# awsaf49/vip-cup-2022

Hardware: AMD Instinct MI355X
Metric: images/sec (200x200, full ensemble) (higher is better)
Workload: dtype f16; 1 GPU; ensemble8; precision=fast, distinct_images=5120, global_batch=256, parallelism=image-parallel dp1, one all-gather of scores, member_streams=3

## Files before the change

### vip-cup-2022_amd/csrc/mlp_fused.hip

```cpp
#include "common.hpp"

namespace {

struct MlpArgs {
    const f16* x;
    const f16* w1;
    const float* b1;
    const f16* w2;
    const float* b2;
    const f16* res;
    f16* y;
    const float* ln_g;
    const float* ln_b;
    float ln_eps;
    int M, Hd;
    int ldx, ldy, ldr, ldw1, ldw2;
    long x_bytes, y_bytes, res_bytes;
    int s1, s2;
    int n_tiles;
};

__device__ __forceinline__ int frag_channel(int j) {
    const int t = (j >> 4) & 1, r = j & 15;
    return (j & ~31) + (r >> 2) * 8 + t * 4 + (r & 3);
}


template <int CK>
__device__ __forceinline__ void ln_fragments(U4H8 (&xf)[CK], const float* __restrict__ g, const float* __restrict__ b,
                                             float eps, int lq) {
    constexpr int C = 32 * CK;
    float v[CK][8];
    float sum = 0.f;
#pragma unroll
    for (int ks = 0; ks < CK; ++ks)
#pragma unroll
        for (int j = 0; j < 8; ++j) {
            v[ks][j] = (float)xf[ks].e[j];
            sum += v[ks][j];
        }
    sum += __shfl_xor(sum, 16, 64);
    sum += __shfl_xor(sum, 32, 64);
    const float mean = sum / (float)C;
    float sq = 0.f;
#pragma unroll
    for (int ks = 0; ks < CK; ++ks)
#pragma unroll
        for (int j = 0; j < 8; ++j) {
            const float d = v[ks][j] - mean;
            sq += d * d;
        }
    sq += __shfl_xor(sq, 16, 64);
    sq += __shfl_xor(sq, 32, 64);
    const float rstd = rsqrtf(sq / (float)C + eps);
#pragma unroll
    for (int ks = 0; ks < CK; ++ks) {
        const float4 g0 = *reinterpret_cast<const float4*>(g + ks * 32 + lq * 8), g1 = *reinterpret_cast<const float4*>(g + ks * 32 + lq * 8 + 4);
        const float4 b0 = *reinterpret_cast<const float4*>(b + ks * 32 + lq * 8), b1 = *reinterpret_cast<const float4*>(b + ks * 32 + lq * 8 + 4);
        const float gg[8] = {g0.x, g0.y, g0.z, g0.w, g1.x, g1.y, g1.z, g1.w};
        const float bb[8] = {b0.x, b0.y, b0.z, b0.w, b1.x, b1.y, b1.z, b1.w};
#pragma unroll
        for (int j = 0; j < 8; ++j) xf[ks].e[j] = (f16)((v[ks][j] - mean) * rstd * gg[j] + bb[j]);
    }
}

template <int CK, int ACT, int PT>
__global__ __launch_bounds__(2048 / PT, 1) void mlp_fused_kernel(MlpArgs a) {
    constexpr int C = 32 * CK, NCT = C / 16, NTHR = 2048 / PT;
    constexpr unsigned OOB = 0xFFFFFFF0u;
    extern __shared__ __attribute__((aligned(16))) char smem[];
    char* w1s = smem;
    char* w2s = smem + a.Hd * a.s1;

    const int tid = threadIdx.x, lane = tid & 63, wave = tid >> 6;
    const int l15 = lane & 15, lq = lane >> 4;

    {
        const __amdgpu_buffer_rsrc_t r1 = __builtin_amdgcn_make_buffer_rsrc((void*)a.w1, 0, (unsigned)(2L * a.Hd * a.ldw1), 0x00020000);
        const __amdgpu_buffer_rsrc_t r2 = __builtin_amdgcn_make_buffer_rsrc((void*)a.w2, 0, (unsigned)(2L * C * a.ldw2), 0x00020000);
        constexpr int cpr1 = CK * 4;
        for (int i = tid; i < a.Hd * cpr1; i += NTHR) {
            const int j = i / cpr1, c = i - j * cpr1;
            const uint4 v = __builtin_bit_cast(
                uint4, __builtin_amdgcn_raw_buffer_load_b128(r1, (unsigned)((frag_channel(j) * a.ldw1 + c * 8) * 2), 0, 0));
            *reinterpret_cast<uint4*>(w1s + j * a.s1 + c * 16) = v;
        }
        const int cpr2 = a.Hd >> 3;
        for (int i = tid; i < C * cpr2; i += NTHR) {
            const int j = i / cpr2, c = i - j * cpr2;
            const uint4 v = __builtin_bit_cast(
                uint4, __builtin_amdgcn_raw_buffer_load_b128(r2, (unsigned)((frag_channel(j) * a.ldw2 + c * 8) * 2), 0, 0));
            *reinterpret_cast<uint4*>(w2s + j * a.s2 + c * 16) = v;
        }
    }
    __syncthreads();

    const __amdgpu_buffer_rsrc_t rx = __builtin_amdgcn_make_buffer_rsrc((void*)a.x, 0, (unsigned)a.x_bytes, 0x00020000);
    const __amdgpu_buffer_rsrc_t rr = __builtin_amdgcn_make_buffer_rsrc((void*)a.res, 0, a.res ? (unsigned)a.res_bytes : 0u, 0x00020000);
    const __amdgpu_buffer_rsrc_t ry = __builtin_amdgcn_make_buffer_rsrc((void*)a.y, 0, (unsigned)a.y_bytes, 0x00020000);
    const __amdgpu_buffer_rsrc_t rb1 = __builtin_amdgcn_make_buffer_rsrc((void*)a.b1, 0, a.b1 ? (unsigned)(a.Hd * 4) : 0u, 0x00020000);
    const __amdgpu_buffer_rsrc_t rb2 = __builtin_amdgcn_make_buffer_rsrc((void*)a.b2, 0, a.b2 ? (unsigned)(C * 4) : 0u, 0x00020000);
    const char* w1l = w1s + l15 * a.s1 + lq * 16;
    const char* w2l = w2s + l15 * a.s2 + lq * 16;
    const int nq = a.Hd >> 5;

    for (int tile = blockIdx.x; tile < a.n_tiles; tile += gridDim.x) {
        const int m0 = tile * 512 + wave * (16 * PT);
        U4H8 xf[CK][PT];
#pragma unroll
        for (int ks = 0; ks < CK; ++ks)
#pragma unroll
            for (int p = 0; p < PT; ++p) {
                const int m = m0 + p * 16 + l15;
                xf[ks][p].u = __builtin_bit_cast(
                    uint4, __builtin_amdgcn_raw_buffer_load_b128(rx, m < a.M ? (unsigned)((m * a.ldx + ks * 32 + lq * 8) * 2) : OOB, 0, 0));
            }
        if (a.ln_g) {
#pragma unroll
            for (int p = 0; p < PT; ++p) {
                U4H8 col[CK];
#pragma unroll
                for (int ks = 0; ks < CK; ++ks) col[ks] = xf[ks][p];
                ln_fragments<CK>(col, a.ln_g, a.ln_b, a.ln_eps, lq);
#pragma unroll
                for (int ks = 0; ks < CK; ++ks) xf[ks][p] = col[ks];
            }
        }
        f32x4 acc2[NCT][PT];
#pragma unroll
        for (int ct = 0; ct < NCT; ++ct) {
            const f32x4 bv = __builtin_bit_cast(
                f32x4, __builtin_amdgcn_raw_buffer_load_b128(rb2, (unsigned)(((ct >> 1) * 32 + lq * 8 + (ct & 1) * 4) * 4), 0, 0));
#pragma unroll
            for (int p = 0; p < PT; ++p) acc2[ct][p] = bv;
        }

        auto gemm1 = [&](int q, f32x4 (&acc1)[2][PT]) {
#pragma unroll
            for (int t = 0; t < 2; ++t) {
                const f32x4 bv = __builtin_bit_cast(
                    f32x4, __builtin_amdgcn_raw_buffer_load_b128(rb1, (unsigned)((q * 32 + lq * 8 + t * 4) * 4), 0, 0));
#pragma unroll
                for (int p = 0; p < PT; ++p) acc1[t][p] = bv;
            }
#pragma unroll
            for (int ks = 0; ks < CK; ++ks)
#pragma unroll
                for (int t = 0; t < 2; ++t) {
                    U4H8 wf;
                    wf.u = *reinterpret_cast<const uint4*>(w1l + (q * 32 + t * 16) * a.s1 + ks * 64);
#pragma unroll
                    for (int p = 0; p < PT; ++p)
                        acc1[t][p] = __builtin_amdgcn_mfma_f32_16x16x32_f16(wf.h, xf[ks][p].h, acc1[t][p], 0, 0, 0);
                }
        };
        auto act_pack = [&](const f32x4 (&acc1)[2][PT], U4H8 (&hf)[PT]) {
#pragma unroll
            for (int p = 0; p < PT; ++p)
#pragma unroll
                for (int t = 0; t < 2; ++t)
#pragma unroll
                    for (int j = 0; j < 4; j += 2) {
                        const f32x2 v = vip_act2<ACT>((f32x2){acc1[t][p][j], acc1[t][p][j + 1]});
                        hf[p].e[t * 4 + j] = (f16)v.x;
                        hf[p].e[t * 4 + j + 1] = (f16)v.y;
                    }
        };
        auto gemm2 = [&](int q, const U4H8 (&hf)[PT]) {
#pragma unroll
            for (int ct = 0; ct < NCT; ++ct) {
                U4H8 wf;
                wf.u = *reinterpret_cast<const uint4*>(w2l + ct * 16 * a.s2 + q * 64);
#pragma unroll
                for (int p = 0; p < PT; ++p)
                    acc2[ct][p] = __builtin_amdgcn_mfma_f32_16x16x32_f16(wf.h, hf[p].h, acc2[ct][p], 0, 0, 0);
            }
        };
        U4H8 hf[PT];
#pragma unroll 1
        for (int q = 0; q < nq; ++q) {
            f32x4 h0[2][PT];
            gemm1(q, h0);
            act_pack(h0, hf);
            gemm2(q, hf);
        }

#pragma unroll
        for (int p = 0; p < PT; ++p) {
            const int m = m0 + p * 16 + l15;
            const bool ok = m < a.M;
#pragma unroll
            for (int hh = 0; hh < CK; ++hh) {
                const int n = hh * 32 + lq * 8;
                U4H8 r;
                r.u = __builtin_bit_cast(uint4, __builtin_amdgcn_raw_buffer_load_b128(
                                                    rr, ok ? (unsigned)((m * a.ldr + n) * 2) : OOB, 0, 0));
                U4H8 o;
#pragma unroll
                for (int j = 0; j < 8; j += 2) {
                    const f32x4 av = acc2[2 * hh + (j >> 2)][p];
                    const f32x2 v = (f32x2){av[j & 3], av[(j & 3) + 1]} + (f32x2){(float)r.e[j], (float)r.e[j + 1]};
                    o.e[j] = (f16)v.x;
                    o.e[j + 1] = (f16)v.y;
                }
                __builtin_amdgcn_raw_buffer_store_b128(
                    __builtin_bit_cast(__attribute__((__vector_size__(4 * sizeof(unsigned)))) unsigned, o.u), ry,
                    ok ? (unsigned)((m * a.ldy + n) * 2) : OOB, 0, 0);
            }
        }
    }
}

static int mlp_stride(int chunks) {
    while ((chunks & 3) != 2) ++chunks;
    return chunks * 16;
}

static int mlp_cu_count() {
    static int n_cu = 0;
    if (!n_cu) {
        int dev = 0;
        hipDeviceProp_t prop;
        if (hipGetDevice(&dev) == hipSuccess && hipGetDeviceProperties(&prop, dev) == hipSuccess) n_cu = prop.multiProcessorCount;
        if (n_cu <= 0) n_cu = 256;
    }
    return n_cu;
}

struct MlpPlan {
    int s1, s2;
    size_t smem;
    int tile;
    int n_tiles;
    int grid;
};

static bool mlp_plan_resident(int C, int M, int Hd, MlpPlan& p) {
    p.s1 = mlp_stride(C / 8);
    p.s2 = mlp_stride(Hd >> 3);
    p.smem = (size_t)Hd * p.s1 + (size_t)C * p.s2;
    if (p.smem > 160 * 1024) return false;
    p.tile = 512;
    p.n_tiles = (M + 511) / 512;
    const int n_cu = mlp_cu_count();
    p.grid = p.n_tiles < n_cu ? p.n_tiles : n_cu;
    return true;
}

static void mlp_plan_stream(int C, int M, MlpPlan& p) {
    p.s1 = mlp_stride(C / 8);
    p.s2 = mlp_stride(4);
    p.smem = 2 * ((size_t)32 * p.s1 + (size_t)C * p.s2);
    p.tile = 256;
    p.n_tiles = (M + 255) / 256;
    const int n_cu = mlp_cu_count();
    p.grid = p.n_tiles < n_cu ? p.n_tiles : n_cu;
}

template <int CK>
int launch_mlp(MlpArgs a, hipStream_t s) {
    MlpPlan p;
    if (!mlp_plan_resident(32 * CK, a.M, a.Hd, p)) return 1;
    a.s1 = p.s1;
    a.s2 = p.s2;
    a.n_tiles = p.n_tiles;
    static bool attr_set = false;
    if (!attr_set) {
        (void)hipFuncSetAttribute(reinterpret_cast<const void*>(mlp_fused_kernel<CK, VIP_ACT_GELU, 2>),
                                  hipFuncAttributeMaxDynamicSharedMemorySize, 160 * 1024);
        attr_set = true;
    }
    hipLaunchKernelGGL((mlp_fused_kernel<CK, VIP_ACT_GELU, 2>), dim3(p.grid), dim3(1024), p.smem, s, a);
    return vip_launch_status("vip_mlp_fused_f16");
}


template <int CK, int ACT>
__global__ __launch_bounds__(512, 1) void mlp_stream_kernel(MlpArgs a) {
    constexpr int C = 32 * CK, PT = 2, NCT = C / 16, NTHR = 512;
    constexpr int W_IT = C / 64;
    constexpr unsigned OOB = 0xFFFFFFF0u;
    extern __shared__ __attribute__((aligned(16))) char smem[];
    const int stage_bytes = 32 * a.s1 + C * a.s2;

    const int tid = threadIdx.x, lane = tid & 63, wave = tid >> 6;
    const int l15 = lane & 15, lq = lane >> 4;

    const __amdgpu_buffer_rsrc_t rx = __builtin_amdgcn_make_buffer_rsrc((void*)a.x, 0, (unsigned)a.x_bytes, 0x00020000);
    const __amdgpu_buffer_rsrc_t rr = __builtin_amdgcn_make_buffer_rsrc((void*)a.res, 0, a.res ? (unsigned)a.res_bytes : 0u, 0x00020000);
    const __amdgpu_buffer_rsrc_t ry = __builtin_amdgcn_make_buffer_rsrc((void*)a.y, 0, (unsigned)a.y_bytes, 0x00020000);
    const __amdgpu_buffer_rsrc_t rb1 = __builtin_amdgcn_make_buffer_rsrc((void*)a.b1, 0, a.b1 ? (unsigned)(a.Hd * 4) : 0u, 0x00020000);
    const __amdgpu_buffer_rsrc_t rb2 = __builtin_amdgcn_make_buffer_rsrc((void*)a.b2, 0, a.b2 ? (unsigned)(C * 4) : 0u, 0x00020000);

    const char* w_ptr[W_IT];
    unsigned w_step[W_IT];
    int w_dst[W_IT];
#pragma unroll
    for (int i = 0; i < W_IT; ++i) {
        const int idx = tid + NTHR * i;
        if (idx < 4 * C) {
            const int row = idx / (C / 8), c = idx - row * (C / 8);
            w_ptr[i] = reinterpret_cast<const char*>(a.w1) + ((long)frag_channel(row) * a.ldw1 + c * 8) * 2;
            w_step[i] = (unsigned)(32 * a.ldw1 * 2);
            w_dst[i] = row * a.s1 + c * 16;
        } else {
            const int j = idx - 4 * C, row = j >> 2, c = j & 3;
            w_ptr[i] = reinterpret_cast<const char*>(a.w2) + ((long)frag_channel(row) * a.ldw2 + c * 8) * 2;
            w_step[i] = 64u;
            w_dst[i] = 32 * a.s1 + row * a.s2 + c * 16;
        }
    }
    uint4 wst[W_IT];
    auto load_w = [&](int q) {
#pragma unroll
        for (int i = 0; i < W_IT; ++i) wst[i] = *reinterpret_cast<const uint4*>(w_ptr[i] + (size_t)q * w_step[i]);
    };
    auto store_w = [&](int buf) {
#pragma unroll
        for (int i = 0; i < W_IT; ++i) *reinterpret_cast<uint4*>(smem + buf * stage_bytes + w_dst[i]) = wst[i];
    };

    const int nq = a.Hd >> 5;
    load_w(0);
    store_w(0);
    __syncthreads();
    int buf = 0;

    for (int tile = blockIdx.x; tile < a.n_tiles; tile += gridDim.x) {
        const int m0 = tile * (NTHR / 64 * 16 * PT) + wave * (16 * PT);
        U4H8 xf[CK][PT];
#pragma unroll
        for (int ks = 0; ks < CK; ++ks)
#pragma unroll
            for (int p = 0; p < PT; ++p) {
                const int m = m0 + p * 16 + l15;
                xf[ks][p].u = __builtin_bit_cast(
                    uint4, __builtin_amdgcn_raw_buffer_load_b128(rx, m < a.M ? (unsigned)((m * a.ldx + ks * 32 + lq * 8) * 2) : OOB, 0, 0));
            }
        if (a.ln_g) {
#pragma unroll
            for (int p = 0; p < PT; ++p) {
                U4H8 col[CK];
#pragma unroll
                for (int ks = 0; ks < CK; ++ks) col[ks] = xf[ks][p];
                ln_fragments<CK>(col, a.ln_g, a.ln_b, a.ln_eps, lq);
#pragma unroll
                for (int ks = 0; ks < CK; ++ks) xf[ks][p] = col[ks];
            }
        }
        f32x4 acc2[NCT][PT];
#pragma unroll
        for (int ct = 0; ct < NCT; ++ct) {
            const f32x4 bv = __builtin_bit_cast(
                f32x4, __builtin_amdgcn_raw_buffer_load_b128(rb2, (unsigned)(((ct >> 1) * 32 + lq * 8 + (ct & 1) * 4) * 4), 0, 0));
#pragma unroll
            for (int p = 0; p < PT; ++p) acc2[ct][p] = bv;
        }

#pragma unroll 1
        for (int q = 0; q < nq; ++q) {
            load_w(q + 1 < nq ? q + 1 : 0);
            __builtin_amdgcn_sched_barrier(0);
            const char* w1l = smem + buf * stage_bytes + l15 * a.s1 + lq * 16;
            const char* w2l = smem + buf * stage_bytes + 32 * a.s1 + l15 * a.s2 + lq * 16;
            f32x4 acc1[2][PT];
#pragma unroll
            for (int t = 0; t < 2; ++t) {
                const f32x4 bv = __builtin_bit_cast(
                    f32x4, __builtin_amdgcn_raw_buffer_load_b128(rb1, (unsigned)((q * 32 + lq * 8 + t * 4) * 4), 0, 0));
#pragma unroll
                for (int p = 0; p < PT; ++p) acc1[t][p] = bv;
            }
#pragma unroll
            for (int ks = 0; ks < CK; ++ks)
#pragma unroll
                for (int t = 0; t < 2; ++t) {
                    U4H8 wf;
                    wf.u = *reinterpret_cast<const uint4*>(w1l + t * 16 * a.s1 + ks * 64);
#pragma unroll
                    for (int p = 0; p < PT; ++p)
                        acc1[t][p] = __builtin_amdgcn_mfma_f32_16x16x32_f16(wf.h, xf[ks][p].h, acc1[t][p], 0, 0, 0);
                }
            U4H8 hf[PT];
#pragma unroll
            for (int p = 0; p < PT; ++p)
#pragma unroll
                for (int t = 0; t < 2; ++t)
#pragma unroll
                    for (int j = 0; j < 4; j += 2) {
                        const f32x2 v = vip_act2<ACT>((f32x2){acc1[t][p][j], acc1[t][p][j + 1]});
                        hf[p].e[t * 4 + j] = (f16)v.x;
                        hf[p].e[t * 4 + j + 1] = (f16)v.y;
                    }
#pragma unroll
            for (int ct = 0; ct < NCT; ++ct) {
                U4H8 wf;
                wf.u = *reinterpret_cast<const uint4*>(w2l + ct * 16 * a.s2);
#pragma unroll
                for (int p = 0; p < PT; ++p)
                    acc2[ct][p] = __builtin_amdgcn_mfma_f32_16x16x32_f16(wf.h, hf[p].h, acc2[ct][p], 0, 0, 0);
            }
            __builtin_amdgcn_sched_barrier(0);
            store_w(buf ^ 1);
            __syncthreads();
            buf ^= 1;
        }

#pragma unroll
        for (int p = 0; p < PT; ++p) {
            const int m = m0 + p * 16 + l15;
            const bool ok = m < a.M;
#pragma unroll
            for (int hh = 0; hh < CK; ++hh) {
                const int n = hh * 32 + lq * 8;
                U4H8 r;
                r.u = __builtin_bit_cast(uint4, __builtin_amdgcn_raw_buffer_load_b128(
                                                    rr, ok ? (unsigned)((m * a.ldr + n) * 2) : OOB, 0, 0));
                U4H8 o;
#pragma unroll
                for (int j = 0; j < 8; j += 2) {
                    const f32x4 av = acc2[2 * hh + (j >> 2)][p];
                    const f32x2 v = (f32x2){av[j & 3], av[(j & 3) + 1]} + (f32x2){(float)r.e[j], (float)r.e[j + 1]};
                    o.e[j] = (f16)v.x;
                    o.e[j + 1] = (f16)v.y;
                }
                __builtin_amdgcn_raw_buffer_store_b128(
                    __builtin_bit_cast(__attribute__((__vector_size__(4 * sizeof(unsigned)))) unsigned, o.u), ry,
                    ok ? (unsigned)((m * a.ldy + n) * 2) : OOB, 0, 0);
            }
        }
    }
}

template <int CK>
int launch_mlp_stream(MlpArgs a, hipStream_t s) {
    MlpPlan p;
    mlp_plan_stream(32 * CK, a.M, p);
    a.s1 = p.s1;
    a.s2 = p.s2;
    a.n_tiles = p.n_tiles;
    static bool attr_set = false;
    if (!attr_set) {
        (void)hipFuncSetAttribute(reinterpret_cast<const void*>(mlp_stream_kernel<CK, VIP_ACT_GELU>),
                                  hipFuncAttributeMaxDynamicSharedMemorySize, 160 * 1024);
        attr_set = true;
    }
    hipLaunchKernelGGL((mlp_stream_kernel<CK, VIP_ACT_GELU>), dim3(p.grid), dim3(512), p.smem, s, a);
    return vip_launch_status("vip_mlp_fused_f16(stream)");
}

}

extern "C" int vip_mlp_fused_supported(int M, int C, int hidden, int act) {
    if (act != VIP_ACT_GELU || hidden % 32 != 0 || hidden <= 0 || M < 8192) return 0;
    if (C == 192) return 1;
    if (C != 64 && C != 96) return 0;
    const long s1 = mlp_stride(C / 8), s2 = mlp_stride(hidden >> 3);
    return (long)hidden * s1 + (long)C * s2 <= 160 * 1024;
}

extern "C" int vip_mlp_fused_plan(int M, int C, int hidden, int act, int* workgroups, int* tile_rows) {
    if (!vip_mlp_fused_supported(M, C, hidden, act)) return 0;
    MlpPlan p;
    if (C == 192) mlp_plan_stream(C, M, p);
    else if (!mlp_plan_resident(C, M, hidden, p)) return 0;
    if (workgroups) *workgroups = p.grid;
    if (tile_rows) *tile_rows = p.tile;
    return p.n_tiles;
}

extern "C" int vip_mlp_fused_f16(const void* x, const float* ln_gamma, const float* ln_beta, float ln_eps, const void* w1,
                                 const float* b1, const void* w2, const float* b2, const void* residual, void* y, int M,
                                 int C, int hidden, int ldx, int ldw1, int ldw2, int ldy, int ldr, int act, void* stream) {
    VIP_REQUIRE(x && w1 && w2 && y, VIP_ERR_BAD_ARG, "vip_mlp_fused_f16: null pointer");
    VIP_REQUIRE((ln_gamma == nullptr) == (ln_beta == nullptr), VIP_ERR_BAD_ARG,
                "vip_mlp_fused_f16: ln_gamma and ln_beta must both be given or both be NULL");
    VIP_REQUIRE(M > 0 && C > 0 && hidden > 0, VIP_ERR_BAD_ARG, "vip_mlp_fused_f16: non-positive dimension");
    VIP_REQUIRE(vip_mlp_fused_supported(M, C, hidden, act), VIP_ERR_UNSUPPORTED,
                "vip_mlp_fused_f16: unsupported shape/activation (C=%d hidden=%d act=%d M=%d); use two vip_gemm_bias_act_f16 calls",
                C, hidden, act, M);
    VIP_REQUIRE(ldx % 8 == 0 && ldy % 8 == 0 && ldw1 % 8 == 0 && ldw2 % 8 == 0 && (!residual || ldr % 8 == 0),
                VIP_ERR_ALIGNMENT, "vip_mlp_fused_f16: leading dimensions must be multiples of 8 halfs");
    VIP_REQUIRE(ldx >= C && ldy >= C && ldw1 >= C && ldw2 >= hidden && (!residual || ldr >= C), VIP_ERR_BAD_ARG,
                "vip_mlp_fused_f16: leading dimension smaller than the row extent");
    MlpArgs a;
    a.x = (const f16*)x; a.w1 = (const f16*)w1; a.b1 = b1; a.w2 = (const f16*)w2; a.b2 = b2;
    a.res = (const f16*)residual; a.y = (f16*)y;
    a.ln_g = ln_gamma; a.ln_b = ln_beta; a.ln_eps = ln_eps;
    a.M = M; a.Hd = hidden; a.ldx = ldx; a.ldy = ldy; a.ldr = ldr; a.ldw1 = ldw1; a.ldw2 = ldw2;
    a.x_bytes = 2L * M * ldx; a.y_bytes = 2L * M * ldy; a.res_bytes = 2L * M * ldr;
    VIP_REQUIRE(a.x_bytes < 0xFFFFFFF0L && a.y_bytes < 0xFFFFFFF0L && a.res_bytes < 0xFFFFFFF0L, VIP_ERR_UNSUPPORTED,
                "vip_mlp_fused_f16: tensor exceeds the 4 GiB buffer-addressing range");
    a.s1 = a.s2 = a.n_tiles = 0;
    int st = 1;
    if (C == 64) st = launch_mlp<2>(a, (hipStream_t)stream);
    else if (C == 96) st = launch_mlp<3>(a, (hipStream_t)stream);
    else if (C == 128) st = launch_mlp_stream<4>(a, (hipStream_t)stream);
    else if (C == 192) st = launch_mlp_stream<6>(a, (hipStream_t)stream);
    else if (C == 256) st = launch_mlp_stream<8>(a, (hipStream_t)stream);
    VIP_REQUIRE(st != 1, VIP_ERR_UNSUPPORTED, "vip_mlp_fused_f16: weights do not fit in LDS");
    return st;
}
```

Measured before the change: 4943 images/sec.

## Stage MLP biases and LN params in LDS and double-buffer weight fragment reads

Biases (and LayerNorm gamma/beta in the resident kernel) are copied once into shared memory, placed in the padding of the weight rows, and read from there instead of issuing global buffer loads on every tile and every hidden chunk. The weight-fragment LDS reads in both GEMMs are double-buffered so the next fragment load is issued before the current MFMAs, overlapping LDS latency with matrix work. Strides become compile-time constants, and the streaming kernel's per-chunk weight staging pointers are advanced incrementally in named registers. The trade-off is more LDS use (with new capacity checks that can reject some shapes), extra registers, and dependence on row padding being large enough to hold the bias data.

Measured after the change: 5009 images/sec, median of 6. 1.3% higher.

```diff
diff --git a/vip-cup-2022_amd/csrc/mlp_fused.hip b/vip-cup-2022_amd/csrc/mlp_fused.hip
--- a/vip-cup-2022_amd/csrc/mlp_fused.hip
+++ b/vip-cup-2022_amd/csrc/mlp_fused.hip
@@ -20,6 +20,11 @@
     int n_tiles;
 };
 
+__host__ __device__ constexpr int mlp_stride(int chunks) {
+    while ((chunks & 3) != 2) ++chunks;
+    return chunks * 16;
+}
+
 __device__ __forceinline__ int frag_channel(int j) {
     const int t = (j >> 4) & 1, r = j & 15;
     return (j & ~31) + (r >> 2) * 8 + t * 4 + (r & 3);
@@ -27,8 +32,7 @@
 
 
 template <int CK>
-__device__ __forceinline__ void ln_fragments(U4H8 (&xf)[CK], const float* __restrict__ g, const float* __restrict__ b,
-                                             float eps, int lq) {
+__device__ __forceinline__ void ln_fragments(U4H8 (&xf)[CK], const char* g, const char* b, int step, float eps, int lq) {
     constexpr int C = 32 * CK;
     float v[CK][8];
     float sum = 0.f;
@@ -55,8 +59,9 @@
     const float rstd = rsqrtf(sq / (float)C + eps);
 #pragma unroll
     for (int ks = 0; ks < CK; ++ks) {
-        const float4 g0 = *reinterpret_cast<const float4*>(g + ks * 32 + lq * 8), g1 = *reinterpret_cast<const float4*>(g + ks * 32 + lq * 8 + 4);
-        const float4 b0 = *reinterpret_cast<const float4*>(b + ks * 32 + lq * 8), b1 = *reinterpret_cast<const float4*>(b + ks * 32 + lq * 8 + 4);
+        const char *gp = g + (ks * 4 + lq) * step, *bp = b + (ks * 4 + lq) * step;
+        const float4 g0 = *reinterpret_cast<const float4*>(gp), g1 = *reinterpret_cast<const float4*>(gp + 16);
+        const float4 b0 = *reinterpret_cast<const float4*>(bp), b1 = *reinterpret_cast<const float4*>(bp + 16);
         const float gg[8] = {g0.x, g0.y, g0.z, g0.w, g1.x, g1.y, g1.z, g1.w};
         const float bb[8] = {b0.x, b0.y, b0.z, b0.w, b1.x, b1.y, b1.z, b1.w};
 #pragma unroll
@@ -67,15 +72,34 @@
 template <int CK, int ACT, int PT>
 __global__ __launch_bounds__(2048 / PT, 1) void mlp_fused_kernel(MlpArgs a) {
     constexpr int C = 32 * CK, NCT = C / 16, NTHR = 2048 / PT;
+    constexpr int S1 = mlp_stride(C / 8);
+    constexpr bool AHEAD = CK != 3;
     constexpr unsigned OOB = 0xFFFFFFF0u;
     extern __shared__ __attribute__((aligned(16))) char smem[];
     char* w1s = smem;
-    char* w2s = smem + a.Hd * a.s1;
+    char* w2s = smem + a.Hd * S1;
 
     const int tid = threadIdx.x, lane = tid & 63, wave = tid >> 6;
     const int l15 = lane & 15, lq = lane >> 4;
 
+    char* b1p = w1s + 2 * C;
+    char* b2p = w2s + 2 * a.Hd;
+    char* lgp = b2p + (C / 8) * a.s2;
+    char* lbp = lgp + (C / 8) * a.s2;
     {
+        const __amdgpu_buffer_rsrc_t rb1 = __builtin_amdgcn_make_buffer_rsrc((void*)a.b1, 0, a.b1 ? (unsigned)(a.Hd * 4) : 0u, 0x00020000);
+        const __amdgpu_buffer_rsrc_t rb2 = __builtin_amdgcn_make_buffer_rsrc((void*)a.b2, 0, a.b2 ? (unsigned)(C * 4) : 0u, 0x00020000);
+        for (int i = tid; i < a.Hd; i += NTHR)
+            *reinterpret_cast<float*>(b1p + ((i & ~31) + ((i >> 3) & 3)) * S1 + (i & 7) * 4) =
+                __builtin_bit_cast(float, __builtin_amdgcn_raw_buffer_load_b32(rb1, (unsigned)(i * 4), 0, 0));
+        for (int i = tid; i < C; i += NTHR) {
+            *reinterpret_cast<float*>(b2p + (i >> 3) * a.s2 + (i & 7) * 4) =
+                __builtin_bit_cast(float, __builtin_amdgcn_raw_buffer_load_b32(rb2, (unsigned)(i * 4), 0, 0));
+            if (a.ln_g) {
+                *reinterpret_cast<float*>(lgp + (i >> 3) * a.s2 + (i & 7) * 4) = a.ln_g[i];
+                *reinterpret_cast<float*>(lbp + (i >> 3) * a.s2 + (i & 7) * 4) = a.ln_b[i];
+            }
+        }
         const __amdgpu_buffer_rsrc_t r1 = __builtin_amdgcn_make_buffer_rsrc((void*)a.w1, 0, (unsigned)(2L * a.Hd * a.ldw1), 0x00020000);
         const __amdgpu_buffer_rsrc_t r2 = __builtin_amdgcn_make_buffer_rsrc((void*)a.w2, 0, (unsigned)(2L * C * a.ldw2), 0x00020000);
         constexpr int cpr1 = CK * 4;
@@ -83,7 +107,7 @@
             const int j = i / cpr1, c = i - j * cpr1;
             const uint4 v = __builtin_bit_cast(
                 uint4, __builtin_amdgcn_raw_buffer_load_b128(r1, (unsigned)((frag_channel(j) * a.ldw1 + c * 8) * 2), 0, 0));
-            *reinterpret_cast<uint4*>(w1s + j * a.s1 + c * 16) = v;
+            *reinterpret_cast<uint4*>(w1s + j * S1 + c * 16) = v;
         }
         const int cpr2 = a.Hd >> 3;
         for (int i = tid; i < C * cpr2; i += NTHR) {
@@ -98,10 +122,9 @@
     const __amdgpu_buffer_rsrc_t rx = __builtin_amdgcn_make_buffer_rsrc((void*)a.x, 0, (unsigned)a.x_bytes, 0x00020000);
     const __amdgpu_buffer_rsrc_t rr = __builtin_amdgcn_make_buffer_rsrc((void*)a.res, 0, a.res ? (unsigned)a.res_bytes : 0u, 0x00020000);
     const __amdgpu_buffer_rsrc_t ry = __builtin_amdgcn_make_buffer_rsrc((void*)a.y, 0, (unsigned)a.y_bytes, 0x00020000);
-    const __amdgpu_buffer_rsrc_t rb1 = __builtin_amdgcn_make_buffer_rsrc((void*)a.b1, 0, a.b1 ? (unsigned)(a.Hd * 4) : 0u, 0x00020000);
-    const __amdgpu_buffer_rsrc_t rb2 = __builtin_amdgcn_make_buffer_rsrc((void*)a.b2, 0, a.b2 ? (unsigned)(C * 4) : 0u, 0x00020000);
-    const char* w1l = w1s + l15 * a.s1 + lq * 16;
+    const char* w1l = w1s + l15 * S1 + lq * 16;
     const char* w2l = w2s + l15 * a.s2 + lq * 16;
+    const char* b1l = b1p + lq * S1;
     const int nq = a.Hd >> 5;
 
     for (int tile = blockIdx.x; tile < a.n_tiles; tile += gridDim.x) {
@@ -115,13 +138,15 @@
                 xf[ks][p].u = __builtin_bit_cast(
                     uint4, __builtin_amdgcn_raw_buffer_load_b128(rx, m < a.M ? (unsigned)((m * a.ldx + ks * 32 + lq * 8) * 2) : OOB, 0, 0));
             }
+        int lqh = lq;
+        asm volatile("" : "+v"(lqh));
         if (a.ln_g) {
 #pragma unroll
             for (int p = 0; p < PT; ++p) {
                 U4H8 col[CK];
 #pragma unroll
                 for (int ks = 0; ks < CK; ++ks) col[ks] = xf[ks][p];
-                ln_fragments<CK>(col, a.ln_g, a.ln_b, a.ln_eps, lq);
+                ln_fragments<CK>(col, lgp, lbp, a.s2, a.ln_eps, lqh);
 #pragma unroll
                 for (int ks = 0; ks < CK; ++ks) xf[ks][p] = col[ks];
             }
@@ -129,30 +154,30 @@
         f32x4 acc2[NCT][PT];
 #pragma unroll
         for (int ct = 0; ct < NCT; ++ct) {
-            const f32x4 bv = __builtin_bit_cast(
-                f32x4, __builtin_amdgcn_raw_buffer_load_b128(rb2, (unsigned)(((ct >> 1) * 32 + lq * 8 + (ct & 1) * 4) * 4), 0, 0));
+            const f32x4 bv = *reinterpret_cast<const f32x4*>(b2p + ((ct >> 1) * 4 + lqh) * a.s2 + (ct & 1) * 16);
 #pragma unroll
             for (int p = 0; p < PT; ++p) acc2[ct][p] = bv;
         }
 
+        U4H8 wf[2];
         auto gemm1 = [&](int q, f32x4 (&acc1)[2][PT]) {
 #pragma unroll
             for (int t = 0; t < 2; ++t) {
-                const f32x4 bv = __builtin_bit_cast(
-                    f32x4, __builtin_amdgcn_raw_buffer_load_b128(rb1, (unsigned)((q * 32 + lq * 8 + t * 4) * 4), 0, 0));
+                const f32x4 bv = *reinterpret_cast<const f32x4*>(b1l + q * 32 * S1 + t * 16);
 #pragma unroll
                 for (int p = 0; p < PT; ++p) acc1[t][p] = bv;
             }
-#pragma unroll
-            for (int ks = 0; ks < CK; ++ks)
-#pragma unroll
-                for (int t = 0; t < 2; ++t) {
-                    U4H8 wf;
-                    wf.u = *reinterpret_cast<const uint4*>(w1l + (q * 32 + t * 16) * a.s1 + ks * 64);
-#pragma unroll
-                    for (int p = 0; p < PT; ++p)
-                        acc1[t][p] = __builtin_amdgcn_mfma_f32_16x16x32_f16(wf.h, xf[ks][p].h, acc1[t][p], 0, 0, 0);
-                }
+            auto rd1 = [&](int f) { return *reinterpret_cast<const uint4*>(w1l + (q * 32 + (f & 1) * 16) * S1 + (f >> 1) * 64); };
+            if constexpr (AHEAD) wf[0].u = rd1(0);
+#pragma unroll
+            for (int f = 0; f < 2 * CK; ++f) {
+                const int ks = f >> 1, t = f & 1, g = f + 1;
+                if constexpr (AHEAD) wf[g & 1].u = g < 2 * CK ? rd1(g) : *reinterpret_cast<const uint4*>(w2l + q * 64);
+                else wf[f & 1].u = rd1(f);
+#pragma unroll
+                for (int p = 0; p < PT; ++p)
+                    acc1[t][p] = __builtin_amdgcn_mfma_f32_16x16x32_f16(wf[f & 1].h, xf[ks][p].h, acc1[t][p], 0, 0, 0);
+            }
         };
         auto act_pack = [&](const f32x4 (&acc1)[2][PT], U4H8 (&hf)[PT]) {
 #pragma unroll
@@ -169,11 +194,11 @@
         auto gemm2 = [&](int q, const U4H8 (&hf)[PT]) {
 #pragma unroll
             for (int ct = 0; ct < NCT; ++ct) {
-                U4H8 wf;
-                wf.u = *reinterpret_cast<const uint4*>(w2l + ct * 16 * a.s2 + q * 64);
+                if constexpr (!AHEAD) wf[ct & 1].u = *reinterpret_cast<const uint4*>(w2l + ct * 16 * a.s2 + q * 64);
+                else if (ct + 1 < NCT) wf[(ct + 1) & 1].u = *reinterpret_cast<const uint4*>(w2l + (ct + 1) * 16 * a.s2 + q * 64);
 #pragma unroll
                 for (int p = 0; p < PT; ++p)
-                    acc2[ct][p] = __builtin_amdgcn_mfma_f32_16x16x32_f16(wf.h, hf[p].h, acc2[ct][p], 0, 0, 0);
+                    acc2[ct][p] = __builtin_amdgcn_mfma_f32_16x16x32_f16(wf[ct & 1].h, hf[p].h, acc2[ct][p], 0, 0, 0);
             }
         };
         U4H8 hf[PT];
@@ -211,11 +236,6 @@
     }
 }
 
-static int mlp_stride(int chunks) {
-    while ((chunks & 3) != 2) ++chunks;
-    return chunks * 16;
-}
-
 static int mlp_cu_count() {
     static int n_cu = 0;
     if (!n_cu) {
@@ -239,7 +259,7 @@
     p.s1 = mlp_stride(C / 8);
     p.s2 = mlp_stride(Hd >> 3);
     p.smem = (size_t)Hd * p.s1 + (size_t)C * p.s2;
-    if (p.smem > 160 * 1024) return false;
+    if (p.smem > 160 * 1024 || p.s1 - 2 * C < 32 || p.s2 - 2 * Hd < 32) return false;
     p.tile = 512;
     p.n_tiles = (M + 511) / 512;
     const int n_cu = mlp_cu_count();
@@ -247,14 +267,20 @@
     return true;
 }
 
-static void mlp_plan_stream(int C, int M, MlpPlan& p) {
+static size_t mlp_stream_lds(int C, int Hd) {
+    return 2 * ((size_t)32 * mlp_stride(C / 8) + (size_t)C * mlp_stride(4)) + 4 * ((size_t)Hd + (size_t)C);
+}
+
+static bool mlp_plan_stream(int C, int M, int Hd, MlpPlan& p) {
     p.s1 = mlp_stride(C / 8);
     p.s2 = mlp_stride(4);
-    p.smem = 2 * ((size_t)32 * p.s1 + (size_t)C * p.s2);
+    p.smem = mlp_stream_lds(C, Hd);
+    if (p.smem > 160 * 1024) return false;
     p.tile = 256;
     p.n_tiles = (M + 255) / 256;
     const int n_cu = mlp_cu_count();
     p.grid = p.n_tiles < n_cu ? p.n_tiles : n_cu;
+    return true;
 }
 
 template <int CK>
@@ -279,9 +305,13 @@
 __global__ __launch_bounds__(512, 1) void mlp_stream_kernel(MlpArgs a) {
     constexpr int C = 32 * CK, PT = 2, NCT = C / 16, NTHR = 512;
     constexpr int W_IT = C / 64;
+    static_assert(W_IT >= 1 && W_IT <= 4, "staging registers are named for up to four chunks");
     constexpr unsigned OOB = 0xFFFFFFF0u;
     extern __shared__ __attribute__((aligned(16))) char smem[];
-    const int stage_bytes = 32 * a.s1 + C * a.s2;
+    constexpr int S1 = mlp_stride(C / 8), S2 = mlp_stride(4);
+    constexpr int stage_bytes = 32 * S1 + C * S2;
+    float* b1s = reinterpret_cast<float*>(smem + 2 * stage_bytes);
+    float* b2s = b1s + a.Hd;
 
     const int tid = threadIdx.x, lane = tid & 63, wave = tid >> 6;
     const int l15 = lane & 15, lq = lane >> 4;
@@ -289,42 +319,66 @@
     const __amdgpu_buffer_rsrc_t rx = __builtin_amdgcn_make_buffer_rsrc((void*)a.x, 0, (unsigned)a.x_bytes, 0x00020000);
     const __amdgpu_buffer_rsrc_t rr = __builtin_amdgcn_make_buffer_rsrc((void*)a.res, 0, a.res ? (unsigned)a.res_bytes : 0u, 0x00020000);
     const __amdgpu_buffer_rsrc_t ry = __builtin_amdgcn_make_buffer_rsrc((void*)a.y, 0, (unsigned)a.y_bytes, 0x00020000);
-    const __amdgpu_buffer_rsrc_t rb1 = __builtin_amdgcn_make_buffer_rsrc((void*)a.b1, 0, a.b1 ? (unsigned)(a.Hd * 4) : 0u, 0x00020000);
-    const __amdgpu_buffer_rsrc_t rb2 = __builtin_amdgcn_make_buffer_rsrc((void*)a.b2, 0, a.b2 ? (unsigned)(C * 4) : 0u, 0x00020000);
-
-    const char* w_ptr[W_IT];
-    unsigned w_step[W_IT];
-    int w_dst[W_IT];
-#pragma unroll
-    for (int i = 0; i < W_IT; ++i) {
+    {
+        const __amdgpu_buffer_rsrc_t rb1 = __builtin_amdgcn_make_buffer_rsrc((void*)a.b1, 0, a.b1 ? (unsigned)(a.Hd * 4) : 0u, 0x00020000);
+        const __amdgpu_buffer_rsrc_t rb2 = __builtin_amdgcn_make_buffer_rsrc((void*)a.b2, 0, a.b2 ? (unsigned)(C * 4) : 0u, 0x00020000);
+        for (int i = tid; i < a.Hd; i += NTHR)
+            b1s[i] = __builtin_bit_cast(float, __builtin_amdgcn_raw_buffer_load_b32(rb1, (unsigned)(i * 4), 0, 0));
+        for (int i = tid; i < C; i += NTHR)
+            b2s[i] = __builtin_bit_cast(float, __builtin_amdgcn_raw_buffer_load_b32(rb2, (unsigned)(i * 4), 0, 0));
+    }
+
+    const char *wp0 = nullptr, *wp1 = nullptr, *wp2 = nullptr, *wp3 = nullptr;
+    unsigned ws0 = 0, ws1 = 0, ws2 = 0, ws3 = 0;
+    int wd0 = 0, wd1 = 0, wd2 = 0, wd3 = 0;
+    auto plan_w = [&](int i, const char*& wp, unsigned& ws, int& wd) {
         const int idx = tid + NTHR * i;
         if (idx < 4 * C) {
             const int row = idx / (C / 8), c = idx - row * (C / 8);
-            w_ptr[i] = reinterpret_cast<const char*>(a.w1) + ((long)frag_channel(row) * a.ldw1 + c * 8) * 2;
-            w_step[i] = (unsigned)(32 * a.ldw1 * 2);
-            w_dst[i] = row * a.s1 + c * 16;
+            wp = reinterpret_cast<const char*>(a.w1) + ((long)frag_channel(row) * a.ldw1 + c * 8) * 2;
+            ws = (unsigned)(32 * a.ldw1 * 2);
+            wd = row * S1 + c * 16;
         } else {
             const int j = idx - 4 * C, row = j >> 2, c = j & 3;
-            w_ptr[i] = reinterpret_cast<const char*>(a.w2) + ((long)frag_channel(row) * a.ldw2 + c * 8) * 2;
-            w_step[i] = 64u;
-            w_dst[i] = 32 * a.s1 + row * a.s2 + c * 16;
-        }
-    }
-    uint4 wst[W_IT];
-    auto load_w = [&](int q) {
-#pragma unroll
-        for (int i = 0; i < W_IT; ++i) wst[i] = *reinterpret_cast<const uint4*>(w_ptr[i] + (size_t)q * w_step[i]);
+            wp = reinterpret_cast<const char*>(a.w2) + ((long)frag_channel(row) * a.ldw2 + c * 8) * 2;
+            ws = 64u;
+            wd = 32 * S1 + row * S2 + c * 16;
+        }
+    };
+    plan_w(0, wp0, ws0, wd0);
+    if constexpr (W_IT > 1) plan_w(1, wp1, ws1, wd1);
+    if constexpr (W_IT > 2) plan_w(2, wp2, ws2, wd2);
+    if constexpr (W_IT > 3) plan_w(3, wp3, ws3, wd3);
+    const int nq = a.Hd >> 5;
+    uint4 wn0, wn1, wn2, wn3;
+    int nxt = 0;
+    auto load_w = [&]() {
+        wn0 = *reinterpret_cast<const uint4*>(wp0);
+        if constexpr (W_IT > 1) wn1 = *reinterpret_cast<const uint4*>(wp1);
+        if constexpr (W_IT > 2) wn2 = *reinterpret_cast<const uint4*>(wp2);
+        if constexpr (W_IT > 3) wn3 = *reinterpret_cast<const uint4*>(wp3);
+        const bool wrap = nxt + 1 >= nq;
+        auto adv = [&](const char*& wp, unsigned ws) { wp += wrap ? -(long)(ws * (unsigned)nxt) : (long)ws; };
+        adv(wp0, ws0);
+        if constexpr (W_IT > 1) adv(wp1, ws1);
+        if constexpr (W_IT > 2) adv(wp2, ws2);
+        if constexpr (W_IT > 3) adv(wp3, ws3);
+        nxt = wrap ? 0 : nxt + 1;
     };
     auto store_w = [&](int buf) {
-#pragma unroll
-        for (int i = 0; i < W_IT; ++i) *reinterpret_cast<uint4*>(smem + buf * stage_bytes + w_dst[i]) = wst[i];
+        char* st = smem + buf * stage_bytes;
+        *reinterpret_cast<uint4*>(st + wd0) = wn0;
+        if constexpr (W_IT > 1) *reinterpret_cast<uint4*>(st + wd1) = wn1;
+        if constexpr (W_IT > 2) *reinterpret_cast<uint4*>(st + wd2) = wn2;
+        if constexpr (W_IT > 3) *reinterpret_cast<uint4*>(st + wd3) = wn3;
     };
 
-    const int nq = a.Hd >> 5;
-    load_w(0);
+    load_w();
     store_w(0);
     __syncthreads();
     int buf = 0;
+    const float* b1l = b1s + lq * 8;
+    const float* b2l = b2s + lq * 8;
 
     for (int tile = blockIdx.x; tile < a.n_tiles; tile += gridDim.x) {
         const int m0 = tile * (NTHR / 64 * 16 * PT) + wave * (16 * PT);
@@ -343,7 +397,7 @@
                 U4H8 col[CK];
 #pragma unroll
                 for (int ks = 0; ks < CK; ++ks) col[ks] = xf[ks][p];
-                ln_fragments<CK>(col, a.ln_g, a.ln_b, a.ln_eps, lq);
+                ln_fragments<CK>(col, reinterpret_cast<const char*>(a.ln_g), reinterpret_cast<const char*>(a.ln_b), 32, a.ln_eps, lq);
 #pragma unroll
                 for (int ks = 0; ks < CK; ++ks) xf[ks][p] = col[ks];
             }
@@ -351,36 +405,35 @@
         f32x4 acc2[NCT][PT];
 #pragma unroll
         for (int ct = 0; ct < NCT; ++ct) {
-            const f32x4 bv = __builtin_bit_cast(
-                f32x4, __builtin_amdgcn_raw_buffer_load_b128(rb2, (unsigned)(((ct >> 1) * 32 + lq * 8 + (ct & 1) * 4) * 4), 0, 0));
+            const f32x4 bv = *reinterpret_cast<const f32x4*>(b2l + (ct >> 1) * 32 + (ct & 1) * 4);
 #pragma unroll
             for (int p = 0; p < PT; ++p) acc2[ct][p] = bv;
         }
 
 #pragma unroll 1
         for (int q = 0; q < nq; ++q) {
-            load_w(q + 1 < nq ? q + 1 : 0);
+            load_w();
             __builtin_amdgcn_sched_barrier(0);
-            const char* w1l = smem + buf * stage_bytes + l15 * a.s1 + lq * 16;
-            const char* w2l = smem + buf * stage_bytes + 32 * a.s1 + l15 * a.s2 + lq * 16;
+            const char* w1l = smem + buf * stage_bytes + l15 * S1 + lq * 16;
+            const char* w2l = w1l + 32 * S1 + l15 * (S2 - S1);
             f32x4 acc1[2][PT];
 #pragma unroll
             for (int t = 0; t < 2; ++t) {
-                const f32x4 bv = __builtin_bit_cast(
-                    f32x4, __builtin_amdgcn_raw_buffer_load_b128(rb1, (unsigned)((q * 32 + lq * 8 + t * 4) * 4), 0, 0));
+                const f32x4 bv = *reinterpret_cast<const f32x4*>(b1l + q * 32 + t * 4);
 #pragma unroll
                 for (int p = 0; p < PT; ++p) acc1[t][p] = bv;
             }
-#pragma unroll
-            for (int ks = 0; ks < CK; ++ks)
-#pragma unroll
-                for (int t = 0; t < 2; ++t) {
-                    U4H8 wf;
-                    wf.u = *reinterpret_cast<const uint4*>(w1l + t * 16 * a.s1 + ks * 64);
-#pragma unroll
-                    for (int p = 0; p < PT; ++p)
-                        acc1[t][p] = __builtin_amdgcn_mfma_f32_16x16x32_f16(wf.h, xf[ks][p].h, acc1[t][p], 0, 0, 0);
-                }
+            U4H8 wf[2];
+            wf[0].u = *reinterpret_cast<const uint4*>(w1l);
+#pragma unroll
+            for (int f = 0; f < 2 * CK; ++f) {
+                const int ks = f >> 1, t = f & 1, g = f + 1;
+                wf[g & 1].u = g < 2 * CK ? *reinterpret_cast<const uint4*>(w1l + (g & 1) * 16 * S1 + (g >> 1) * 64)
+                                         : *reinterpret_cast<const uint4*>(w2l);
+#pragma unroll
+                for (int p = 0; p < PT; ++p)
+                    acc1[t][p] = __builtin_amdgcn_mfma_f32_16x16x32_f16(wf[f & 1].h, xf[ks][p].h, acc1[t][p], 0, 0, 0);
+            }
             U4H8 hf[PT];
 #pragma unroll
             for (int p = 0; p < PT; ++p)
@@ -394,11 +447,10 @@
                     }
 #pragma unroll
             for (int ct = 0; ct < NCT; ++ct) {
-                U4H8 wf;
-                wf.u = *reinterpret_cast<const uint4*>(w2l + ct * 16 * a.s2);
+                if (ct + 1 < NCT) wf[(ct + 1) & 1].u = *reinterpret_cast<const uint4*>(w2l + (ct + 1) * 16 * S2);
 #pragma unroll
                 for (int p = 0; p < PT; ++p)
-                    acc2[ct][p] = __builtin_amdgcn_mfma_f32_16x16x32_f16(wf.h, hf[p].h, acc2[ct][p], 0, 0, 0);
+                    acc2[ct][p] = __builtin_amdgcn_mfma_f32_16x16x32_f16(wf[ct & 1].h, hf[p].h, acc2[ct][p], 0, 0, 0);
             }
             __builtin_amdgcn_sched_barrier(0);
             store_w(buf ^ 1);
@@ -435,7 +487,7 @@
 template <int CK>
 int launch_mlp_stream(MlpArgs a, hipStream_t s) {
     MlpPlan p;
-    mlp_plan_stream(32 * CK, a.M, p);
+    if (!mlp_plan_stream(32 * CK, a.M, a.Hd, p)) return 1;
     a.s1 = p.s1;
     a.s2 = p.s2;
     a.n_tiles = p.n_tiles;
@@ -453,7 +505,8 @@
 
 extern "C" int vip_mlp_fused_supported(int M, int C, int hidden, int act) {
     if (act != VIP_ACT_GELU || hidden % 32 != 0 || hidden <= 0 || M < 8192) return 0;
-    if (C == 192) return 1;
+    if (C == 192)
+        return mlp_stream_lds(C, hidden) <= 160 * 1024;
     if (C != 64 && C != 96) return 0;
     const long s1 = mlp_stride(C / 8), s2 = mlp_stride(hidden >> 3);
     return (long)hidden * s1 + (long)C * s2 <= 160 * 1024;
@@ -462,8 +515,9 @@
 extern "C" int vip_mlp_fused_plan(int M, int C, int hidden, int act, int* workgroups, int* tile_rows) {
     if (!vip_mlp_fused_supported(M, C, hidden, act)) return 0;
     MlpPlan p;
-    if (C == 192) mlp_plan_stream(C, M, p);
-    else if (!mlp_plan_resident(C, M, hidden, p)) return 0;
+    if (C == 192) {
+        if (!mlp_plan_stream(C, M, hidden, p)) return 0;
+    } else if (!mlp_plan_resident(C, M, hidden, p)) return 0;
     if (workgroups) *workgroups = p.grid;
     if (tile_rows) *tile_rows = p.tile;
     return p.n_tiles;
```
